# VachaLab/gorder

Hardware: AMD Instinct MI355X
Metric: trajectory frames/sec (higher is better)
Workload: dtype f32

## Files before the change

gorder_amd/abi.py:

```python
from __future__ import annotations

import ctypes as C
import os
from dataclasses import dataclass, field
from typing import List, Optional, Sequence

import numpy as np

_HERE = os.path.dirname(os.path.abspath(__file__))
LIB_PATH = os.environ.get("GORDER_HIP_LIB") or os.path.join(_HERE, "libgorder_hip.so")

OK = 0
ERR_UNDEFINED_BOX = 1
ERR_NOT_ORTHOGONAL_BOX = 2
ERR_ZERO_BOX = 3
ERR_UNDEFINED_POSITION = 4
ERR_INVALID_GLOBAL_MEMBRANE_CENTER = 5
ERR_INVALID_LOCAL_MEMBRANE_CENTER = 6
ERR_INVALID_ARGUMENT = 100
ERR_DEVICE = 101
ERR_NO_DEVICE = 102
ERR_BOX_RANGE = 103
ERR_LEAFLETS_NOT_PRIMED = 104
ERR_OVERFLOW = 105
# ... 235 lines not shown
        ge = self.geometry
        grp = _u32(ge.group) if ge.group is not None else None
        t.geometry.kind = ge.kind
        t.geometry.invert = 1 if ge.invert else 0
        t.geometry.reference = ge.reference
        t.geometry.point[:] = [float(x) for x in ge.point]
        t.geometry.n_group = 0 if grp is None else grp.size
        t.geometry.group = _ptr(grp)
        t.geometry.xdim[:] = [float(x) for x in ge.xdim]
        t.geometry.ydim[:] = [float(x) for x in ge.ydim]
        t.geometry.zdim[:] = [float(x) for x in ge.zdim]
        t.geometry.radius = ge.radius
        t.geometry.span[:] = [float(x) for x in ge.span]
        t.geometry.orientation = ge.orientation
        t.geometry.structure_box[:] = [float(x) for x in ge.structure_box]
        dn = self.dynamic_normal
        cloud = _u32(dn.cloud) if dn.cloud is not None else None
        t.dynamic_normal.enabled = 1 if dn.enabled else 0
        t.dynamic_normal.radius = dn.radius
        t.dynamic_normal.n_cloud = 0 if cloud is None else cloud.size
        t.dynamic_normal.cloud = _ptr(cloud)
        keep += [mts, mem, grp, cloud]
        return t, keep


_EXPORTS = [
    "gorder_hip_create", "gorder_hip_destroy", "gorder_hip_n_accumulators", "gorder_hip_ordermap_dims",
    "gorder_hip_set_stream", "gorder_hip_submit_device", "gorder_hip_submit_host",
    "gorder_hip_prime_leaflets", "gorder_hip_set_manual_leaflets", "gorder_hip_synchronize",
    "gorder_hip_finish", "gorder_hip_timewise", "gorder_hip_leaflets", "gorder_hip_leaflet_distances",
    "gorder_hip_normals", "gorder_hip_export_maps", "gorder_hip_set_normals",
    "gorder_hip_accumulators_device", "gorder_hip_bind_accumulators", "gorder_hip_last_error_index", "gorder_hip_last_error_frame", "gorder_hip_kernel_time_names",
    "gorder_hip_last_error_message", "gorder_hip_strerror", "gorder_hip_kernel_time", "gorder_hip_kernel_time_group", "gorder_hip_plan",
    "gorder_hip_plan_tables", "gorder_hip_selftest_arithmetic", "gorder_hip_selftest_trig", "gorder_hip_run_trajectory",
    "gorder_hip_comm_unique_id", "gorder_hip_comm_create", "gorder_hip_comm_destroy", "gorder_hip_allreduce",
    "gorder_hip_reset", "gorder_hip_xtc_decode", "gorder_hip_release_staging", "gorder_hip_speculation_stats", "gorder_hip_local_decide_stats",
]

_lib = None


class GorderHipError(RuntimeError):
    def __init__(self, status: int, message: str = "", index: int = 0, frame: int = 0):
        self.status = status
        self.index = index
        self.frame = frame
        super().__init__(f"gorder_hip status {status}: {message}")


def load_library() -> C.CDLL:
    global _lib
    if _lib is not None:
        return _lib
    if not os.path.exists(LIB_PATH):
        raise GorderHipError(ERR_NO_DEVICE, f"{LIB_PATH} is missing: run `python -c 'import __graft_entry__ as g; "
                                            "g.build()'` (there is no CPU fallback)")
    try:
        import torch
        _rt = os.path.join(os.path.dirname(torch.__file__), "lib", "libamdhip64.so")
        if os.path.exists(_rt):
            C.CDLL(_rt, mode=C.RTLD_GLOBAL)
    except ImportError:
        pass
    lib = C.CDLL(LIB_PATH)
    vp, u32, u64, i32 = C.c_void_p, C.c_uint32, C.c_uint64, C.c_int
    lib.gorder_hip_create.argtypes = [C.POINTER(CTables), C.POINTER(vp)]
    lib.gorder_hip_destroy.argtypes = [vp]
# ... 3 lines not shown
    lib.gorder_hip_ordermap_dims.argtypes = [vp, C.POINTER(u32), C.POINTER(u32)]
    lib.gorder_hip_ordermap_dims.restype = u32
    lib.gorder_hip_set_stream.argtypes = [vp, vp]
    lib.gorder_hip_submit_device.argtypes = [vp, vp, vp, vp, u32]
    lib.gorder_hip_submit_host.argtypes = [vp, vp, vp, vp, u32]
    lib.gorder_hip_prime_leaflets.argtypes = [vp, vp, vp, u64]
    lib.gorder_hip_set_manual_leaflets.argtypes = [vp, vp, u64]
    lib.gorder_hip_synchronize.argtypes = [vp]
    lib.gorder_hip_finish.argtypes = [vp, vp, vp, vp, vp, C.POINTER(u64)]
    lib.gorder_hip_timewise.argtypes = [vp, vp, vp, u64]
    lib.gorder_hip_leaflets.argtypes = [vp, vp, C.POINTER(u64)]
    lib.gorder_hip_leaflet_distances.argtypes = [vp, vp]
    lib.gorder_hip_normals.argtypes = [vp, vp, vp]
    lib.gorder_hip_export_maps.argtypes = [vp, vp, vp, u64]
    lib.gorder_hip_set_normals.argtypes = [vp, vp, u32]
    lib.gorder_hip_accumulators_device.argtypes = [vp, C.POINTER(vp), C.POINTER(u64)]
    lib.gorder_hip_bind_accumulators.argtypes = [vp, vp, u64]
    lib.gorder_hip_last_error_index.argtypes = [vp]
    lib.gorder_hip_last_error_index.restype = u64
    lib.gorder_hip_kernel_time_names.argtypes = [vp]
    lib.gorder_hip_kernel_time_names.restype = C.c_char_p
    lib.gorder_hip_last_error_frame.argtypes = [vp]
    lib.gorder_hip_last_error_frame.restype = u64
    lib.gorder_hip_last_error_message.argtypes = [vp]
    lib.gorder_hip_last_error_message.restype = C.c_char_p
    lib.gorder_hip_strerror.argtypes = [i32]
    lib.gorder_hip_strerror.restype = C.c_char_p
    lib.gorder_hip_kernel_time.argtypes = [vp, C.POINTER(C.c_double), C.POINTER(u64), i32]
    lib.gorder_hip_kernel_time_group.argtypes = [vp, C.c_uint32, C.POINTER(C.c_char_p), C.POINTER(C.c_double), C.POINTER(u64)]
    lib.gorder_hip_plan.argtypes = [vp, C.POINTER(CPlan)]
    lib.gorder_hip_speculation_stats.argtypes = [vp, C.POINTER(C.c_uint64)]
    lib.gorder_hip_local_decide_stats.argtypes = [vp, C.POINTER(C.c_uint64)]
    lib.gorder_hip_plan_tables.argtypes = [C.POINTER(CTables), C.POINTER(CPlan), C.POINTER(i32)]
    lib.gorder_hip_selftest_arithmetic.argtypes = [i32, C.c_uint64, C.c_uint64, C.POINTER(C.c_uint64)]
    lib.gorder_hip_selftest_trig.argtypes = [i32, i32, C.c_uint32, C.c_uint32, C.c_uint32, C.c_void_p]
    lib.gorder_hip_run_trajectory.argtypes = [vp, C.POINTER(CTrajectory), C.POINTER(CTrajectoryStats)]
    lib.gorder_hip_comm_unique_id.argtypes = [vp]
    lib.gorder_hip_comm_create.argtypes = [vp, vp, i32, i32, C.POINTER(vp)]
    lib.gorder_hip_comm_destroy.argtypes = [vp]
    lib.gorder_hip_comm_destroy.restype = None
    lib.gorder_hip_allreduce.argtypes = [vp, vp]
    lib.gorder_hip_reset.argtypes = [vp]
    lib.gorder_hip_xtc_decode.argtypes = [vp, vp, u64, vp, u32, u32, vp, u32, vp, u32]
    lib.gorder_hip_release_staging.argtypes = [vp]
    lib.gorder_hip_release_staging.restype = None
    _lib = lib
    return lib


def selftest_trig(fn: str, first_bits: int, stride: int, n: int, device: int = 0) -> np.ndarray:
    lib = load_library()
    out = np.empty(n, dtype=np.float32)
    st = lib.gorder_hip_selftest_trig(device, {"acos": 0, "acos_cores": 1, "cos": 2, "sin": 3}[fn], first_bits, stride, n, out.ctypes.data)
    if st != 0:
        raise GorderHipError(st, "gorder_hip_selftest_trig")
    return out


def selftest_arithmetic(n: int = 1 << 26, seed: int = 1, device: int = 0):
    lib = load_library()
    out = (C.c_uint64 * 2)()
    st = lib.gorder_hip_selftest_arithmetic(device, n, seed, out)
    if st != 0:
        raise GorderHipError(st, lib.gorder_hip_strerror(st).decode())
    return int(out[0]), int(out[1])


def plan_tables(tables: Tables) -> dict:
    lib = load_library()
    ct, keep = tables.as_ctypes()
    plan, check = CPlan(), C.c_int(-1)
    st = lib.gorder_hip_plan_tables(C.byref(ct), C.byref(plan), C.byref(check))
    if st != OK:
        raise GorderHipError(st, lib.gorder_hip_strerror(st).decode())
    d = {name: getattr(plan, name) for name, _ in CPlan._fields_}
    d["selfcheck"] = check.value
    return d


@dataclass
class Results:
    sums: np.ndarray
    counts: np.ndarray
    n_frames: int
    map_sums: Optional[np.ndarray] = None
    map_counts: Optional[np.ndarray] = None

    def order_ticks(self, min_samples: int = 1) -> np.ndarray:
        n = self.counts.astype(np.int64)
        ok = n >= max(1, min_samples)
        q = np.full(self.sums.shape, np.iinfo(np.int64).min, dtype=np.int64)
        q[ok] = (np.abs(self.sums[ok]) // n[ok]) * np.sign(self.sums[ok])
        return q

    def order(self, min_samples: int = 1) -> np.ndarray:
        out = np.full(self.sums.shape, np.nan, dtype=np.float32)
        n = self.counts.astype(np.int64)
        ok = n >= max(1, min_samples)
# ... 248 lines not shown
```

gorder_amd/csrc/gorder_hip.hip:

```cpp
#include <hip/hip_runtime.h>

#include <dlfcn.h>

#include <cmath>
#include <cstdio>
#include <cstdlib>
#include <cstring>
#include <mutex>
#include <new>
#include <string>
#include <deque>
#include <vector>

#include "../../include/gorder_hip.h"
#include "gm_math.h"
#include "plan.h"

#pragma clang fp contract(off)

using gorder::DirectItem;
using gorder::Item;
using gorder::kBlock;
using gorder::Plan;
using gorder::Tile;

#include "kernels_common.h"
#include "kernels_bonds.h"
#include "kernels_extras.h"
#include "kernels_leaflets.h"
#include "kernels_normals.h"
#include "kernels_xtc.h"


struct gorder_hip_handle {
    void *traj_cache = nullptr;
    void (*traj_cache_free)(gorder_hip_handle *) = nullptr;
    Plan plan;
    gorder_tables_t tables{};
    int device = 0;
    hipStream_t own_stream = nullptr;
    hipStream_t stream = nullptr;
    Tile *d_tiles = nullptr;
    Item *d_items = nullptr;
    uint32_t *d_tile_slots = nullptr;
    DirectItem *d_direct = nullptr;
    Tile *d_ua_tiles = nullptr;
    gorder::UaItem *d_ua_items = nullptr;
    uint32_t *d_ua_tile_slots = nullptr;
    uint32_t map_nx = 0, map_ny = 0;
    unsigned long long *d_map_sums = nullptr, *d_map_cnts = nullptr;
    unsigned long long *d_map_packed = nullptr;
    unsigned long long *d_map_rec = nullptr;
    size_t map_rec_cap = 0;
    gorder::MapRun *d_ua_runs = nullptr, *d_runs = nullptr;
// ... 63 lines not shown
    bool spec_enabled = false;
    bool spec_now = false;
    uint2 *d_own = nullptr;
    float4 *d_mom = nullptr;
    size_t mom_cap = 0;
    float *d_head_z = nullptr;
    size_t head_z_cap = 0;
    uint32_t *d_own_head_begin = nullptr;
    uint2 *d_own_heads = nullptr;
    float *d_spec_center = nullptr;
    uint8_t *d_spec_ok = nullptr;
    size_t spec_frames_cap = 0;
    uint32_t *d_spec_counters = nullptr;
    static constexpr uint32_t kSpecRing = 8;
    uint32_t *h_spec_counters = nullptr;
    hipEvent_t spec_counters_copied[kSpecRing] = {};
    uint64_t spec_ring_frames[kSpecRing] = {};
    uint32_t *d_spec_mol_begin = nullptr;
    SpecSample *d_spec_samples = nullptr;
    uint64_t spec_batches = 0, spec_fixed = 0, spec_exact_frames = 0;
    float *d_stage_xyz[2] = {nullptr, nullptr}, *d_stage_box[2] = {nullptr, nullptr};
    size_t stage_xyz_cap[2] = {0, 0}, stage_box_cap[2] = {0, 0};
    hipEvent_t stage_copied[2] = {nullptr, nullptr}, stage_computed[2] = {nullptr, nullptr};
    bool stage_used[2] = {false, false};
    int stage_next = 0;
    hipStream_t copy_stream = nullptr;
    float n2 = 1.0f, n2sq = 1.0f;
    int axis = -1;
    int frames_per_stage = kFramesPerStage;
    bool membrane_is_frame = false;
    bool use_gather = false;
    uint32_t wg_capacity = 256u * 6u;
    uint32_t wg_target = 0;
    uint32_t lw = 0;
    size_t lds_bytes = 0;
    uint64_t n_frames = 0;
    uint64_t err_index = 0;
    std::string err_msg;
    static constexpr uint32_t kTimingEvents = 1024;
    struct TimingSeg { uint32_t label, ev_a, ev_b; };
    bool timing_on = false;
    hipEvent_t timing_ev[kTimingEvents] = {};
    uint32_t timing_next_ev = 0;
    int timing_open_label = -1;
    uint32_t timing_open_ev = 0;
    std::deque<TimingSeg> timing_pending;
    std::vector<std::string> timing_labels;
    std::vector<double> timing_label_ms;
    std::vector<uint64_t> timing_label_n;
    uint64_t timing_launches = 0;
    std::string timed_kernels;
    std::vector<uint32_t> host_heads, host_dyn_heads;
    uint32_t *d_mol_slot0 = nullptr;
    uint64_t err_frame = 0;
    struct BatchLog { uint64_t ordinal, first, stride; std::vector<uint64_t> list; };
    static constexpr size_t kBatchLog = 4096;
    std::deque<BatchLog> batch_log;
    uint64_t n_submits = 0;
    const unsigned long long *decoder_key = nullptr;
};

namespace {

int fail(gorder_hip_handle *h, int status, const std::string &msg) {
    if (h) h->err_msg = msg;
    return status;
// ... 199 lines not shown
    HIP_TRY(h, hipGetLastError());
    h->last_normals.resize(4 * (size_t)n_mol);
    HIP_TRY(h, hipMemcpyAsync(h->last_normals.data(), h->d_dyn_normals + (size_t)(a.n_frames - 1) * n_mol,
                              4 * sizeof(float) * (size_t)n_mol, hipMemcpyDeviceToHost, h->stream));
    return GORDER_OK;
}

int launch_orders(gorder_hip_handle *h, FrameArgs &a) {
    const Plan &p = h->plan;
    const uint32_t n_tiles = (uint32_t)p.tiles.size();
    const bool extras = h->extra.maps || h->extra.tw || h->extra.geom_kind || h->dyn || h->manual_active;
#define name(k) TIMING_MARK(h, k)
    if (h->dyn && !h->manual_active) {
        const int st2 = run_dynamic_normals(h, a);
        if (st2 != GORDER_OK) return st2;
    }
    if (h->extra.geom_kind) {
        int st2;
        if ((st2 = ensure(h, &h->d_shapes, &h->shapes_cap, (size_t)a.n_frames * 8)) != GORDER_OK) return st2;
        const gorder_geometry_t &ge = h->tables.geometry;
        GeomArgs ga{};
        ga.xyz = a.xyz; ga.box9 = a.box9; ga.n_atoms = a.n_atoms; ga.pbc = a.pbc;
        ga.kind = ge.kind; ga.reference = ge.reference; ga.orientation = ge.orientation;
        for (int d = 0; d < 3; d++) { ga.point[d] = ge.point[d]; ga.structure_box[d] = ge.structure_box[d]; }
        for (int d = 0; d < 2; d++) { ga.xdim[d] = ge.xdim[d]; ga.ydim[d] = ge.ydim[d]; ga.zdim[d] = ge.zdim[d]; ga.span[d] = ge.span[d]; }
        ga.radius = ge.radius; ga.group = h->d_geom_group; ga.n_group = ge.n_group;
        ga.shapes = h->d_shapes; ga.err = h->d_err;
        name("k_geom_shapes");
        hipLaunchKernelGGL(k_geom_shapes, dim3(a.n_frames), dim3(256), 0, h->stream, ga);
        HIP_TRY(h, hipGetLastError());
    }
    if (n_tiles && !extras) {
        const uint32_t G = (uint32_t)h->frames_per_stage;
        const uint32_t n_stages = (a.n_frames + G - 1) / G;
        uint32_t target = h->wg_target ? h->wg_target : h->wg_capacity;
        if (!h->wg_target) target = 12u * h->wg_capacity;
        uint32_t n_chunks = std::max(1u, target / n_tiles);
        n_chunks = std::min(n_chunks, std::max(1u, n_stages / 4u));
        uint32_t fpc = ((n_stages + n_chunks - 1) / n_chunks) * G;
        n_chunks = (a.n_frames + fpc - 1) / fpc;
        a.frames_per_chunk = fpc;
        const uint64_t grid = (uint64_t)n_tiles * n_chunks;
        if (grid > 0x7fffffffull) return fail(h, GORDER_ERR_INVALID_ARGUMENT, "batch too large");
        const bool ac = (h->tables.flags & GORDER_FLAG_TRIG_ACOS_COS) != 0;
        const dim3 g((uint32_t)grid), b(kBlock);
#define GORDER_LAUNCH_TILED_A(G_, NPF_, AC_, PBC_, LF_, AX_)                                               \
        do {                                                                                                \
            if (LF_ && h->spec_now)                                                                         \
                hipLaunchKernelGGL((k_bonds_tiled<G_, NPF_, AC_, PBC_, LF_, AX_, LF_>), g, b, h->lds_bytes, h->stream, a, \
                                   a.xyz, a.box9, a.aflags, a.arow, h->d_tiles, h->d_items, h->d_tile_slots, n_tiles, h->lw); \
            else                                                                                            \
                hipLaunchKernelGGL((k_bonds_tiled<G_, NPF_, AC_, PBC_, LF_, AX_>), g, b, h->lds_bytes, h->stream, a,     \
                                   a.xyz, a.box9, a.aflags, a.arow, h->d_tiles, h->d_items, h->d_tile_slots, n_tiles,   \
                                   h->lw);                                                                  \
        } while (0)
#define GORDER_LAUNCH_TILED_V(G_, NPF_, AC_, PBC_, LF_)                                                    \
        do {                                                                                                \
            if (h->axis == 2) GORDER_LAUNCH_TILED_A(G_, NPF_, AC_, PBC_, LF_, 2);                           \
            else if (h->axis == 1) GORDER_LAUNCH_TILED_A(G_, NPF_, AC_, PBC_, LF_, 1);                      \
            else if (h->axis == 0) GORDER_LAUNCH_TILED_A(G_, NPF_, AC_, PBC_, LF_, 0);                      \
            else GORDER_LAUNCH_TILED_A(G_, NPF_, AC_, PBC_, LF_, -1);                                       \
        } while (0)
#define GORDER_LAUNCH_TILED(G_, NPF_)                                                                       \
        do {                                                                                                \
            const int v_ = (ac ? 4 : 0) | (a.pbc ? 2 : 0) | (a.leaflets ? 1 : 0);                           \
            switch (v_) {                                                                                   \
                case 0: GORDER_LAUNCH_TILED_V(G_, NPF_, false, false, false); break;                        \
                case 1: GORDER_LAUNCH_TILED_V(G_, NPF_, false, false, true); break;                         \
                case 2: GORDER_LAUNCH_TILED_V(G_, NPF_, false, true, false); break;                         \
                case 3: GORDER_LAUNCH_TILED_V(G_, NPF_, false, true, true); break;                          \
                case 4: GORDER_LAUNCH_TILED_V(G_, NPF_, true, false, false); break;                         \
                case 5: GORDER_LAUNCH_TILED_V(G_, NPF_, true, false, true); break;                          \
                case 6: GORDER_LAUNCH_TILED_V(G_, NPF_, true, true, false); break;                          \
                default: GORDER_LAUNCH_TILED_V(G_, NPF_, true, true, true); break;                          \
            }                                                                                               \
// ... 349 lines not shown
    if (device < 0 || device >= count || hipSetDevice(device) != hipSuccess) return GORDER_ERR_INVALID_ARGUMENT;
    if (n == 0) return GORDER_OK;
    float *d = nullptr;
    if (hipMalloc((void **)&d, (size_t)n * sizeof(float)) != hipSuccess) return GORDER_ERR_DEVICE;
    hipLaunchKernelGGL(k_selftest_trig, dim3((n + 255u) / 256u), dim3(256), 0, 0, fn, first_bits, stride, n, d);
    int st = GORDER_OK;
    if (hipDeviceSynchronize() != hipSuccess || hipMemcpy(out, d, (size_t)n * sizeof(float), hipMemcpyDeviceToHost) != hipSuccess)
        st = GORDER_ERR_DEVICE;
    (void)hipFree(d);
    return st;
}

int gorder_hip_plan_tables(const gorder_tables_t *tables, gorder_hip_plan_t *out, int *selfcheck) {
    if (!tables || !out) return GORDER_ERR_INVALID_ARGUMENT;
    Plan p;
    const int st = gorder::build_plan(*tables, env_flag("GORDER_HIP_FORCE_DIRECT"), p);
    if (st != GORDER_OK) return st;
    out->n_tiles = (uint32_t)p.tiles.size();
    out->block_threads = kBlock;
    out->max_window_atoms = p.max_window;
    out->n_direct_items = (uint32_t)p.direct.size();
    out->frames_per_stage = kFramesPerStage;
    const uint32_t lw = ((3u * p.max_window + 3u + 3u) / 4u) * 4u;
    size_t lds = (size_t)kFramesPerStage * lw * sizeof(float);
    if (lds < (size_t)kBlock * 24) lds = (size_t)kBlock * 24;
    out->lds_bytes = (uint32_t)lds;
    out->map_staged = 0;
    out->map_lds_bytes = 0;
    out->leaflets_one_read = p.spec_ok ? 1u : 0u;
    if (selfcheck) *selfcheck = gorder::selfcheck_plan(*tables, p);
    return GORDER_OK;
}

int gorder_hip_create(const gorder_tables_t *t, gorder_hip_handle **out) {
    if (!t || !out) return GORDER_ERR_INVALID_ARGUMENT;
    *out = nullptr;
    int n_dev = 0;
    if (hipGetDeviceCount(&n_dev) != hipSuccess || n_dev <= 0) return GORDER_ERR_NO_DEVICE;
    if (t->device < 0 || t->device >= n_dev) return GORDER_ERR_INVALID_ARGUMENT;

    gorder_hip_handle *h = new (std::nothrow) gorder_hip_handle();
    if (!h) return GORDER_ERR_DEVICE;
    *out = h;
    h->tables = *t;
    h->tables.molecule_types = nullptr;
    h->tables.leaflets.membrane = nullptr;
    h->device = t->device;
    HIP_TRY(h, hipSetDevice(h->device));
    if ((t->flags & GORDER_FLAG_UA_FAST_NORMALISE) && (t->flags & GORDER_FLAG_TRIG_ACOS_COS))
        return fail(h, GORDER_ERR_INVALID_ARGUMENT, "GORDER_FLAG_UA_FAST_NORMALISE (tolerance-bounded) and GORDER_FLAG_TRIG_ACOS_COS (literal) exclude each other");
    const bool ua_rows_only = t->timewise && !t->ordermap.enabled && t->geometry.kind == GORDER_GEOM_NONE && !t->dynamic_normal.enabled;
    int st = gorder::build_plan(*t, env_flag("GORDER_HIP_FORCE_DIRECT"), h->plan, !env_flag("GORDER_HIP_UA_SLOT_WAVES") && !ua_rows_only);
    if (st != GORDER_OK) return fail(h, st, "invalid bond tables");
    const Plan &p = h->plan;
    for (uint32_t m = 0; m < t->n_molecule_types; m++)
        h->map_max_mol = std::max(h->map_max_mol, t->molecule_types[m].n_molecules);
    HIP_TRY(h, hipStreamCreateWithFlags(&h->own_stream, hipStreamNonBlocking));
    h->stream = h->own_stream;
    if ((st = upload(h, &h->d_tiles, p.tiles)) != GORDER_OK) return st;
    if ((st = upload(h, &h->d_items, p.items)) != GORDER_OK) return st;
    if ((st = upload(h, &h->d_tile_slots, p.tile_slots)) != GORDER_OK) return st;
    if ((st = upload(h, &h->d_direct, p.direct)) != GORDER_OK) return st;
    if ((st = upload(h, &h->d_ua_tiles, p.ua_tiles)) != GORDER_OK) return st;
    if ((st = upload(h, &h->d_ua_items, p.ua_items)) != GORDER_OK) return st;
    if ((st = upload(h, &h->d_ua_tile_slots, p.ua_tile_slots)) != GORDER_OK) return st;
    {
// ... 65 lines not shown
        }
        if ((e.maps || e.tw || e.geom_kind) && !p.direct.empty())
            return fail(h, GORDER_ERR_INVALID_ARGUMENT,
                        "ordermaps / timewise / geometry need every bond to fit an atom window");
    }
    HIP_TRY(h, hipMalloc((void **)&h->d_err, (kErrWords + 2u) * sizeof(uint32_t)));
    HIP_TRY(h, hipMemset(h->d_err, 0xff, kErrWords * sizeof(uint32_t)));
    HIP_TRY(h, hipMemset(h->d_err + kErrWords, 0, 2u * sizeof(uint32_t)));
    h->acc_words = 4 * (size_t)p.n_acc + 1;
    HIP_TRY(h, hipMalloc((void **)&h->d_acc, h->acc_words * sizeof(unsigned long long)));
    HIP_TRY(h, hipMemset(h->d_acc, 0, h->acc_words * sizeof(unsigned long long)));
    if (const char *e = getenv("GORDER_HIP_MAP_FOLD_LIMIT")) {
        const long v = atol(e);
        if (v >= 2 && (unsigned long long)v <= kMapFoldLimit) h->map_fold_limit = (uint64_t)v;
    }
    if (const char *e = getenv("GORDER_HIP_REPLICAS")) {
        const int r = atoi(e);
        if (r >= 1 && r <= 1024) h->n_rep = (uint32_t)r;
    }
    if (p.n_acc) {
        const size_t rep_bytes = (size_t)h->n_rep * 4u * p.n_acc * sizeof(unsigned long long);
        HIP_TRY(h, hipMalloc((void **)&h->d_rep, rep_bytes));
        HIP_TRY(h, hipMemset(h->d_rep, 0, rep_bytes));
    }
    {
        const float *n = t->normal;
        h->n2sq = (n[0] * n[0] + n[1] * n[1]) + n[2] * n[2];
        h->n2 = sqrtf(h->n2sq);
        for (int d = 0; d < 3; d++)
            if (n[d] == 1.0f && n[(d + 1) % 3] == 0.0f && n[(d + 2) % 3] == 0.0f) h->axis = d;
        h->extra.axis = h->axis;
    }
    if (const char *e = getenv("GORDER_HIP_KERNEL")) h->use_gather = strcmp(e, "gather") == 0;
    if (const char *e = getenv("GORDER_HIP_WG_TARGET")) {
        const int w = atoi(e);
        if (w > 0) h->wg_target = (uint32_t)w;
    }
    h->lw = ((3u * p.max_window + 3u + 3u) / 4u) * 4u;
    h->lds_bytes = (size_t)h->frames_per_stage * h->lw * sizeof(float);
    if (h->lds_bytes < (size_t)kBlock * 24) h->lds_bytes = (size_t)kBlock * 24;
    {
        int n_cu = 256, per_cu = 6;
        (void)hipDeviceGetAttribute(&n_cu, hipDeviceAttributeMultiprocessorCount, h->device);
        const bool ac = (t->flags & GORDER_FLAG_TRIG_ACOS_COS) != 0;
        const hipError_t e = ac ? hipOccupancyMaxActiveBlocksPerMultiprocessor(&per_cu, k_bonds_tiled<4, 5, true, true, false, -1>, kBlock, h->lds_bytes)
                                : hipOccupancyMaxActiveBlocksPerMultiprocessor(&per_cu, k_bonds_tiled<4, 5, false, true, false, 2>, kBlock, h->lds_bytes);
        if (e != hipSuccess || per_cu < 1) per_cu = 4;
        h->wg_capacity = (uint32_t)n_cu * (uint32_t)per_cu;
    }

    const gorder_dynamic_normal_t &dn = t->dynamic_normal;
    if (dn.enabled) {
        if (!(dn.radius > 0.0f)) return fail(h, GORDER_ERR_INVALID_ARGUMENT, "dynamic normals need a positive radius");
        if (!dn.cloud || dn.n_cloud == 0) return fail(h, GORDER_ERR_INVALID_ARGUMENT, "dynamic normals need the NormalHeads group");
        if (!p.direct.empty()) return fail(h, GORDER_ERR_INVALID_ARGUMENT, "dynamic normals: a bond spans more than the LDS window");
        std::vector<uint32_t> cloud(dn.cloud, dn.cloud + dn.n_cloud), nheads;
        for (uint32_t a : cloud)
            if (a >= t->n_atoms) return fail(h, GORDER_ERR_INVALID_ARGUMENT, "NormalHeads index out of range");
        for (uint32_t m = 0; m < t->n_molecule_types; m++) {
            const gorder_moltype_t &mt = t->molecule_types[m];
            if (!mt.normal_heads) return fail(h, GORDER_ERR_INVALID_ARGUMENT, "dynamic normals need normal_heads[] per molecule type");
            for (uint32_t k = 0; k < mt.n_molecules; k++) {
                if (mt.normal_heads[k] >= t->n_atoms) return fail(h, GORDER_ERR_INVALID_ARGUMENT, "normal head index out of range");
                nheads.push_back(mt.normal_heads[k]);
            }
        }
// ... 942 lines not shown
```

gorder_amd/csrc/kernels_bonds.h:

```cpp
#pragma once

namespace {

__device__ __forceinline__ int grid_index(float x, float lo, float bin, uint32_t n, bool core) {
    const float k = __builtin_roundf(core ? gm_div_core(x - lo, bin) : (x - lo) / bin);
    if (!(k >= 0.0f) || !(k < (float)n)) return -1;
    return (int)k;
}
__device__ __forceinline__ int grid_index_fast(float x, float lo, float inv_bin, uint32_t n) {
    const float k = __builtin_floorf(__builtin_fmaf(x - lo, inv_bin, 0.5f));
    if (!(k >= 0.0f) || !(k < (float)n)) return -1;
    return (int)k;
}
constexpr uint32_t kRecFrames = 4;
struct TiledMapOut {
    uint32_t plane;
    float x0, y0, binx, biny;
    uint32_t nx, ny;
    int bin_core;
    unsigned long long *words;
    unsigned long long *ticks;
};
__device__ __forceinline__ unsigned long long tick_sample_word(int tick, bool lower) {
    return ((unsigned long long)(lower ? 1u : 0u) << 32) | (unsigned long long)(uint32_t)tick;
// ... 290 lines not shown
            s += d;
            q = __builtin_fmaf(d, d, q);
            mn = mom_min(mn, z[u]);
            mx = mom_max(mx, z[u]);
        }
    }
#define GORDER_MOM_STEP(CTRL, MASK, CTRL_TEXT)                                                  \
    s += mom_dpp0<CTRL, MASK>(s); q += mom_dpp0<CTRL, MASK>(q);                                 \
    GORDER_MOM_MINMAX_DPP(CTRL_TEXT);
    GORDER_MOM_STEP(0x111, 0xf, "row_shr:1 row_mask:0xf bank_mask:0xf")
    GORDER_MOM_STEP(0x112, 0xf, "row_shr:2 row_mask:0xf bank_mask:0xf")
    GORDER_MOM_STEP(0x114, 0xf, "row_shr:4 row_mask:0xf bank_mask:0xf")
    GORDER_MOM_STEP(0x118, 0xf, "row_shr:8 row_mask:0xf bank_mask:0xf")
    GORDER_MOM_STEP(0x142, 0xa, "row_bcast:15 row_mask:0xa bank_mask:0xf")
    GORDER_MOM_STEP(0x143, 0xc, "row_bcast:31 row_mask:0xc bank_mask:0xf")
#undef GORDER_MOM_STEP
    const bool all_finite = __all(finite);
    if (lane == 63u) a.mom[(size_t)f * n_tiles + tile_id] = make_float4(all_finite ? s : __builtin_nanf(""), q, mn, mx);
    if (my_head.y != 0xffffffffu) a.head_z[(size_t)f * a.n_mol_total + my_head.y] = slot[sh + a.mom_dim + 3u * my_head.x];
}
template <int G, int NPF, bool ACOS_COS, bool PBC, bool LEAF, int AXIS, bool MOM = false>
__global__ __launch_bounds__(kBlock, GORDER_TILED_MIN_WAVES) void k_bonds_tiled(FrameArgs a_in, const float *__restrict__ xyz,
                                                      const float *__restrict__ box9,
                                                      const uint8_t *__restrict__ aflags,
                                                      const uint32_t *__restrict__ arow,
                                                      const Tile *__restrict__ tiles,
                                                      const Item *__restrict__ items,
                                                      const uint32_t *__restrict__ tile_slots,
                                                      uint32_t n_tiles, uint32_t lw) {
    extern __shared__ __attribute__((aligned(16))) float lds[];
    using S = TiledStage<G, NPF, ACOS_COS, PBC, LEAF, AXIS>;
    FrameArgs a = a_in;
    a.xyz = xyz; a.box9 = box9; a.aflags = aflags; a.arow = arow;
    const uint32_t tile_id = blockIdx.x % n_tiles;
    const uint32_t chunk = blockIdx.x / n_tiles;
    const Tile t = tiles[tile_id];
    const uint32_t tid = threadIdx.x;
    const uint32_t sk = tid / S::TPF, si = tid % S::TPF;
    const bool active = tid < t.n_items;
    Item it{0, 0, 0, 0, 0};
    if (active) it = items[t.item0 + tid];

    const uint32_t f_begin = chunk * a.frames_per_chunk;
    const uint32_t f_end = min(a.n_frames, f_begin + a.frames_per_chunk);
    const uint32_t f_full = f_begin + ((f_end - f_begin) / G) * G;

    SampleAcc acc;
    int bad = 0;
    uint32_t nan_which = 0, nan_frame = kNoNan;
    v4f pre[NPF];
    uint2 own = make_uint2(0u, 0u), my_head = make_uint2(0u, 0xffffffffu);
    if (MOM) {
        own = a.own[tile_id];
        const uint32_t hq = a.own_head_begin[tile_id] + (tid & 63u);
        if (hq < a.own_head_begin[tile_id + 1u]) my_head = a.own_heads[hq];
    }

    if (f_begin < f_full) S::template load<false>(a, t, f_begin, f_end, sk, si, pre);
    for (uint32_t f0 = f_begin; f0 < f_full; f0 += G) {
        const bool finite = S::template store<false, MOM>(a, t, f0, f_end, sk, si, pre, lds, lw);
        __syncthreads();
        if (f0 + G < f_full) S::template load<false>(a, t, f0 + G, f_end, sk, si, pre);
        if (MOM) {
            static_assert(!MOM || (uint32_t)G * 64u == kBlock, "a wave per frame slot");
            tiled_moments(a, t, own, tile_id, n_tiles, f0 + sk, lds + (size_t)sk * lw, finite, my_head);
        }
        if (active) S::compute(a, t, it, f0, lds, lw, acc, bad, nan_which, nan_frame);
        __syncthreads();
    }
    if (f_full < f_end) {
        S::template load<true>(a, t, f_full, f_end, sk, si, pre);
        const bool finite = S::template store<true, MOM>(a, t, f_full, f_end, sk, si, pre, lds, lw);
        __syncthreads();
        if (MOM && f_full + sk < f_end) tiled_moments(a, t, own, tile_id, n_tiles, f_full + sk, lds + (size_t)sk * lw, finite, my_head);
        if (active) S::compute_tail(a, t, it, f_full, f_end, lds, lw, acc, bad, nan_which, nan_frame);
        __syncthreads();
    }
// ... 158 lines not shown
```

gorder_amd/csrc/kernels_common.h:

```cpp
#pragma once

namespace {

constexpr int kFramesPerStage = 4;
constexpr uint32_t kErrWords = 8;

struct FrameArgs {
    const float *xyz;
    const float *box9;
    uint32_t n_atoms;
    uint32_t n_frames;
    uint32_t frame0;
    uint32_t frames_per_chunk;
    int pbc;
    float nx, ny, nz, n2, n2sq;
    int leaflets;
    const uint8_t *aflags;
    const uint32_t *arow;
    uint32_t n_mol_total;
    unsigned long long *acc;
    unsigned long long *rep;
    uint32_t n_rep;
    uint32_t n_acc;
    uint32_t *err;
    const uint2 *own;
    float4 *mom;
    int mom_dim;
    const uint32_t *own_head_begin;
    const uint2 *own_heads;
    float *head_z;
};

constexpr unsigned long long kErrNone = ~0ull;
enum ErrStage : uint32_t { kStageBox = 0, kStageSystem = 1, kStageTypes = 2, kStageEnd = 3 };
__device__ __forceinline__ void raise_error(uint32_t *err, uint32_t code, uint32_t frame, uint32_t stage,
                                            uint32_t slot = 0, uint32_t sample = 0, uint32_t mol = 0,
                                            uint32_t detail = 0) {
    const unsigned long long key =
        ((unsigned long long)(code == GORDER_ERR_BOX_RANGE ? 1u : 0u) << 63) |
        ((unsigned long long)min(frame, 0x7fffffu) << 40) | ((unsigned long long)(stage & 3u) << 38) |
        ((unsigned long long)min(slot, 0x3fffu) << 24) | ((unsigned long long)(sample & 1u) << 23) |
        ((unsigned long long)min(mol, 0x1ffffu) << 6) | ((unsigned long long)(detail & 3u) << 4) |
        (unsigned long long)(code == GORDER_ERR_BOX_RANGE ? 8u : (code == GORDER_ERR_TRAJECTORY_FORMAT ? 9u : (code & 15u)));
    atomicMin(reinterpret_cast<unsigned long long *>(err), key);
}
__device__ __forceinline__ void raise_box_range(uint32_t *err, uint32_t frame) {
// ... 99 lines not shown
```

gorder_amd/csrc/plan.h:

```cpp
#pragma once
#include <algorithm>
#include <map>
#include <tuple>
#include <cstdint>
#include <utility>
#include <vector>

#include "../../include/gorder_hip.h"

namespace gorder {

#ifndef GORDER_BLOCK
#define GORDER_BLOCK 256
#endif
constexpr uint32_t kBlock = GORDER_BLOCK;
constexpr uint32_t kMaxWindow = 1024;

struct Item {
    uint16_t li, lj;
    uint16_t lslot;
    uint16_t pad;
    uint32_t mol;
};
struct Tile {
// ... 444 lines not shown
            for (uint32_t j = 0; j < run.n; j++) {
                const Item &it = p.items_by_slot[tile.item0 + run.tid0 + j];
                if (p.tile_slots[tile.slot0 + it.lslot] != sl) return 10;
                if (p.item_run.size() != p.items.size() || p.item_run[tile.item0 + run.tid0 + j] != ((run.tid0 << 16) | run.n))
                    return 16;
                covered[tile.item0 + run.tid0 + j]++;
            }
        }
    for (uint32_t c : covered)
        if (c != 1) return 11;
    if (!p.ua_tiles.empty()) {
        if (p.ua_run_begin.size() != (size_t)p.n_acc + 1) return 12;
        size_t lanes = 0, want_lanes = 0;
        for (const UaItem &it : p.ua_items) want_lanes += it.kind == GORDER_UA_CH3 ? 3 : it.kind == GORDER_UA_CH2 ? 2 : 1;
        for (uint32_t sl = 0; sl < p.n_acc; sl++)
            for (uint32_t r = p.ua_run_begin[sl]; r < p.ua_run_begin[sl + 1]; r++) {
                const MapRun &run = p.ua_runs[r];
                if (run.tile >= p.ua_tiles.size() || run.k > 2 || run.tid0 + run.n > p.ua_tiles[run.tile].n_items) return 13;
                const Tile &tile = p.ua_tiles[run.tile];
                for (uint32_t j = 0; j < run.n; j++) {
                    const UaItem &it = p.ua_items[tile.item0 + run.tid0 + j];
                    if (p.ua_tile_slots[tile.slot0 + it.lslot0 + run.k] != sl) return 14;
                    if (p.ua_item_run.size() != p.ua_items.size() ||
                        p.ua_item_run[tile.item0 + run.tid0 + j] != ((run.tid0 << 16) | run.n))
                        return 17;
                    lanes++;
                }
            }
        if (lanes != want_lanes) return 15;
    }
    return 0;
}

}
```

include/gorder_hip.h:

```cpp
#ifndef GORDER_HIP_H
#define GORDER_HIP_H

#include <stddef.h>
#include <stdint.h>

#include "gorder_xtc.h"

#ifdef __cplusplus
extern "C" {
#endif

typedef enum {
    GORDER_OK = 0,
    GORDER_ERR_UNDEFINED_BOX = 1,
    GORDER_ERR_NOT_ORTHOGONAL_BOX = 2,
    GORDER_ERR_ZERO_BOX = 3,
    GORDER_ERR_UNDEFINED_POSITION = 4,
    GORDER_ERR_INVALID_GLOBAL_MEMBRANE_CENTER = 5,
    GORDER_ERR_INVALID_LOCAL_MEMBRANE_CENTER = 6,
    GORDER_ERR_DYNAMIC_NORMAL = 7,
    GORDER_ERR_INVALID_ARGUMENT = 100,
    GORDER_ERR_DEVICE = 101,
    GORDER_ERR_NO_DEVICE = 102,
    GORDER_ERR_BOX_RANGE = 103,
// ... 176 lines not shown
int gorder_hip_comm_unique_id(uint8_t id[128]);
int gorder_hip_comm_create(gorder_hip_handle *h, const uint8_t id[128], int n_ranks, int rank, void **comm_out);
void gorder_hip_comm_destroy(void *comm);
int gorder_hip_allreduce(gorder_hip_handle *h, void *nccl_comm);

int gorder_hip_reset(gorder_hip_handle *h);

int gorder_hip_export_maps(gorder_hip_handle *h, void *d_sums, void *d_counts, uint64_t n_u64);

int gorder_hip_bind_accumulators(gorder_hip_handle *h, void *d_ptr, uint64_t n_u64);

uint64_t gorder_hip_last_error_index(const gorder_hip_handle *h);
uint64_t gorder_hip_last_error_frame(const gorder_hip_handle *h);
const char *gorder_hip_last_error_message(const gorder_hip_handle *h);
const char *gorder_hip_strerror(int status);

int gorder_hip_kernel_time(gorder_hip_handle *h, double *ms, uint64_t *launches, int reset);
int gorder_hip_kernel_time_group(gorder_hip_handle *h, uint32_t index, const char **name, double *ms, uint64_t *segments);
const char *gorder_hip_kernel_time_names(const gorder_hip_handle *h);

typedef struct {
    uint32_t n_tiles;
    uint32_t block_threads;
    uint32_t max_window_atoms;
    uint32_t n_direct_items;
    uint32_t frames_per_stage;
    uint32_t lds_bytes;
    uint32_t map_staged;
    uint32_t map_lds_bytes;
    uint32_t leaflets_one_read;
} gorder_hip_plan_t;
int gorder_hip_plan(const gorder_hip_handle *h, gorder_hip_plan_t *plan);
int gorder_hip_plan_tables(const gorder_tables_t *tables, gorder_hip_plan_t *plan, int *selfcheck);

int gorder_hip_speculation_stats(gorder_hip_handle *h, uint64_t out[4]);

int gorder_hip_local_decide_stats(gorder_hip_handle *h, uint64_t out[4]);

int gorder_hip_selftest_arithmetic(int device, uint64_t n, uint64_t seed, uint64_t mismatches[2]);
int gorder_hip_selftest_trig(int device, int fn, uint32_t first_bits, uint32_t stride, uint32_t n, float *out);

#ifdef __cplusplus
}
#endif
#endif
```

Measured before the change: 20.94 million.

## Balance tiled kernel chunks across XCDs with grouped work decomposition

Replaces the tile×chunk grid calculation with a scheduler that picks a chunk count that is a multiple of 8 (the XCD count) and minimizes wave-quantization waste against workgroup capacity. Stages are spread evenly, with the first n_long chunks taking one extra stage. Block indices are decoded so that consecutive blocks on different XCDs share a tile. The intent is to cut tail imbalance from uneven chunks and partial waves, and to improve per-XCD cache locality for tile data. The cost is extra integer decode per block and a more complex schedule; a legacy env option and a host-side inspection API are added.

```diff
diff --git a/gorder_amd/abi.py b/gorder_amd/abi.py
--- a/gorder_amd/abi.py
+++ b/gorder_amd/abi.py
@@ -291,7 +291,7 @@
     "gorder_hip_normals", "gorder_hip_export_maps", "gorder_hip_set_normals",
     "gorder_hip_accumulators_device", "gorder_hip_bind_accumulators", "gorder_hip_last_error_index", "gorder_hip_last_error_frame", "gorder_hip_kernel_time_names",
     "gorder_hip_last_error_message", "gorder_hip_strerror", "gorder_hip_kernel_time", "gorder_hip_kernel_time_group", "gorder_hip_plan",
-    "gorder_hip_plan_tables", "gorder_hip_selftest_arithmetic", "gorder_hip_selftest_trig", "gorder_hip_run_trajectory",
+    "gorder_hip_plan_tables", "gorder_hip_tiled_schedule", "gorder_hip_selftest_arithmetic", "gorder_hip_selftest_trig", "gorder_hip_run_trajectory",
     "gorder_hip_comm_unique_id", "gorder_hip_comm_create", "gorder_hip_comm_destroy", "gorder_hip_allreduce",
     "gorder_hip_reset", "gorder_hip_xtc_decode", "gorder_hip_release_staging", "gorder_hip_speculation_stats", "gorder_hip_local_decide_stats",
 ]
@@ -361,6 +361,7 @@
     lib.gorder_hip_speculation_stats.argtypes = [vp, C.POINTER(C.c_uint64)]
     lib.gorder_hip_local_decide_stats.argtypes = [vp, C.POINTER(C.c_uint64)]
     lib.gorder_hip_plan_tables.argtypes = [C.POINTER(CTables), C.POINTER(CPlan), C.POINTER(i32)]
+    lib.gorder_hip_tiled_schedule.argtypes = [u32, u32, u32, u32, i32, vp, vp, u64]
     lib.gorder_hip_selftest_arithmetic.argtypes = [i32, C.c_uint64, C.c_uint64, C.POINTER(C.c_uint64)]
     lib.gorder_hip_selftest_trig.argtypes = [i32, i32, C.c_uint32, C.c_uint32, C.c_uint32, C.c_void_p]
     lib.gorder_hip_run_trajectory.argtypes = [vp, C.POINTER(CTrajectory), C.POINTER(CTrajectoryStats)]
@@ -393,6 +394,23 @@
     if st != 0:
         raise GorderHipError(st, lib.gorder_hip_strerror(st).decode())
     return int(out[0]), int(out[1])
+
+
+def k1_schedule(n_frames: int, n_tiles: int, capacity: int, target: int = 0, legacy: bool = False, launches: bool = False):
+    lib = load_library()
+    info = np.zeros(5, dtype=np.uint32)
+    st = lib.gorder_hip_tiled_schedule(n_frames, n_tiles, capacity, target, int(legacy), info.ctypes.data, None, 0)
+    if st != OK:
+        raise GorderHipError(st, lib.gorder_hip_strerror(st).decode())
+    d = dict(zip(("n_chunks", "stages", "n_long", "grouped", "grid"), (int(v) for v in info)))
+    if launches:
+        out = np.zeros((d["grid"], 3), dtype=np.uint32)
+        st = lib.gorder_hip_tiled_schedule(n_frames, n_tiles, capacity, target, int(legacy), info.ctypes.data,
+                                        out.ctypes.data, d["grid"])
+        if st != OK:
+            raise GorderHipError(st, lib.gorder_hip_strerror(st).decode())
+        d["launches"] = out
+    return d
 
 
 def plan_tables(tables: Tables) -> dict:
diff --git a/gorder_amd/csrc/gorder_hip.hip b/gorder_amd/csrc/gorder_hip.hip
--- a/gorder_amd/csrc/gorder_hip.hip
+++ b/gorder_amd/csrc/gorder_hip.hip
@@ -20,6 +20,7 @@
 
 using gorder::DirectItem;
 using gorder::Item;
+using gorder::k1_decode;
 using gorder::kBlock;
 using gorder::Plan;
 using gorder::Tile;
@@ -149,6 +150,7 @@
     bool use_gather = false;
     uint32_t wg_capacity = 256u * 6u;
     uint32_t wg_target = 0;
+    bool k1_legacy = false;
     uint32_t lw = 0;
     size_t lds_bytes = 0;
     uint64_t n_frames = 0;
@@ -414,15 +416,12 @@
     }
     if (n_tiles && !extras) {
         const uint32_t G = (uint32_t)h->frames_per_stage;
-        const uint32_t n_stages = (a.n_frames + G - 1) / G;
-        uint32_t target = h->wg_target ? h->wg_target : h->wg_capacity;
-        if (!h->wg_target) target = 12u * h->wg_capacity;
-        uint32_t n_chunks = std::max(1u, target / n_tiles);
-        n_chunks = std::min(n_chunks, std::max(1u, n_stages / 4u));
-        uint32_t fpc = ((n_stages + n_chunks - 1) / n_chunks) * G;
-        n_chunks = (a.n_frames + fpc - 1) / fpc;
-        a.frames_per_chunk = fpc;
-        const uint64_t grid = (uint64_t)n_tiles * n_chunks;
+        const uint32_t target = h->wg_target ? h->wg_target : 12u * h->wg_capacity;
+        const gorder::K1Schedule ks = gorder::k1_schedule(a.n_frames, G, n_tiles, h->wg_capacity, target,
+                                                          h->k1_legacy || h->use_gather);
+        a.frames_per_chunk = ks.stages * G;
+        a.n_chunks = ks.n_chunks; a.chunk_stages = ks.stages; a.n_long = ks.n_long; a.grouped = ks.grouped;
+        const uint64_t grid = ks.grid;
         if (grid > 0x7fffffffull) return fail(h, GORDER_ERR_INVALID_ARGUMENT, "batch too large");
         const bool ac = (h->tables.flags & GORDER_FLAG_TRIG_ACOS_COS) != 0;
         const dim3 g((uint32_t)grid), b(kBlock);
@@ -838,6 +837,25 @@
     return GORDER_OK;
 }
 
+int gorder_hip_tiled_schedule(uint32_t n_frames, uint32_t n_tiles, uint32_t capacity, uint32_t target, int legacy,
+                           uint32_t *info, uint32_t *launches, uint64_t max_launches) {
+    if (!info) return GORDER_ERR_INVALID_ARGUMENT;
+    const uint32_t G = kFramesPerStage;
+    const gorder::K1Schedule s = gorder::k1_schedule(n_frames, G, n_tiles, capacity, target ? target : 12u * capacity, legacy != 0);
+    info[0] = s.n_chunks; info[1] = s.stages; info[2] = s.n_long; info[3] = s.grouped;
+    info[4] = (uint32_t)std::min<uint64_t>(s.grid, 0xffffffffu);
+    if (!launches) return GORDER_OK;
+    if (s.grid > max_launches) return GORDER_ERR_INVALID_ARGUMENT;
+    for (uint32_t L = 0; L < (uint32_t)s.grid; L++) {
+        uint32_t tile = 0, f0 = 0, f1 = 0;
+        const bool on = k1_decode(L, n_tiles, G, n_frames, s.n_chunks, s.stages, s.n_long, s.grouped, tile, f0, f1);
+        launches[3u * (size_t)L] = on ? tile : 0xffffffffu;
+        launches[3u * (size_t)L + 1] = f0;
+        launches[3u * (size_t)L + 2] = f1;
+    }
+    return GORDER_OK;
+}
+
 int gorder_hip_create(const gorder_tables_t *t, gorder_hip_handle **out) {
     if (!t || !out) return GORDER_ERR_INVALID_ARGUMENT;
     *out = nullptr;
@@ -969,6 +987,7 @@
         h->extra.axis = h->axis;
     }
     if (const char *e = getenv("GORDER_HIP_KERNEL")) h->use_gather = strcmp(e, "gather") == 0;
+    if (const char *e = getenv("GORDER_HIP_K1_SCHEDULE")) h->k1_legacy = strcmp(e, "legacy") == 0;
     if (const char *e = getenv("GORDER_HIP_WG_TARGET")) {
         const int w = atoi(e);
         if (w > 0) h->wg_target = (uint32_t)w;
diff --git a/gorder_amd/csrc/kernels_bonds.h b/gorder_amd/csrc/kernels_bonds.h
--- a/gorder_amd/csrc/kernels_bonds.h
+++ b/gorder_amd/csrc/kernels_bonds.h
@@ -346,8 +346,10 @@
     using S = TiledStage<G, NPF, ACOS_COS, PBC, LEAF, AXIS>;
     FrameArgs a = a_in;
     a.xyz = xyz; a.box9 = box9; a.aflags = aflags; a.arow = arow;
-    const uint32_t tile_id = blockIdx.x % n_tiles;
-    const uint32_t chunk = blockIdx.x / n_tiles;
+    uint32_t tile_id, f_begin, f_end;
+    if (!k1_decode(blockIdx.x, n_tiles, (uint32_t)G, a.n_frames, a.n_chunks, a.chunk_stages, a.n_long, a.grouped, tile_id,
+                   f_begin, f_end))
+        return;
     const Tile t = tiles[tile_id];
     const uint32_t tid = threadIdx.x;
     const uint32_t sk = tid / S::TPF, si = tid % S::TPF;
@@ -355,8 +357,6 @@
     Item it{0, 0, 0, 0, 0};
     if (active) it = items[t.item0 + tid];
 
-    const uint32_t f_begin = chunk * a.frames_per_chunk;
-    const uint32_t f_end = min(a.n_frames, f_begin + a.frames_per_chunk);
     const uint32_t f_full = f_begin + ((f_end - f_begin) / G) * G;
 
     SampleAcc acc;
diff --git a/gorder_amd/csrc/kernels_common.h b/gorder_amd/csrc/kernels_common.h
--- a/gorder_amd/csrc/kernels_common.h
+++ b/gorder_amd/csrc/kernels_common.h
@@ -12,6 +12,7 @@
     uint32_t n_frames;
     uint32_t frame0;
     uint32_t frames_per_chunk;
+    uint32_t n_chunks, chunk_stages, n_long, grouped;
     int pbc;
     float nx, ny, nz, n2, n2sq;
     int leaflets;
diff --git a/gorder_amd/csrc/plan.h b/gorder_amd/csrc/plan.h
--- a/gorder_amd/csrc/plan.h
+++ b/gorder_amd/csrc/plan.h
@@ -500,4 +500,76 @@
     return 0;
 }
 
-}
+#if defined(__HIP__)
+#define GORDER_HD __host__ __device__
+#else
+#define GORDER_HD
+#endif
+constexpr uint32_t kXcds = 8;
+struct K1Schedule {
+    uint32_t n_chunks = 0;
+    uint32_t stages = 0;
+    uint32_t n_long = 0;
+    uint32_t grouped = 0;
+    uint64_t grid = 0;
+};
+inline uint32_t gcd_u32(uint32_t a, uint32_t b) {
+    while (b) { const uint32_t r = a % b; a = b; b = r; }
+    return a;
+}
+inline K1Schedule k1_schedule(uint32_t n_frames, uint32_t G, uint32_t n_tiles, uint32_t capacity, uint32_t target, bool legacy) {
+    K1Schedule s;
+    if (!n_frames || !n_tiles || !G) return s;
+    const uint32_t n_stages = (n_frames + G - 1) / G;
+    const uint32_t c_max = std::max(1u, n_stages / 4u);
+    const uint32_t c0 = std::min(std::max(1u, target / n_tiles), c_max);
+    const uint64_t cap = std::max(1u, capacity);
+    auto waste = [&](uint32_t c) {
+        const uint64_t wg = (uint64_t)n_tiles * c;
+        return (double)((wg + cap - 1) / cap * cap) / (double)wg;
+    };
+    const uint32_t st = (n_stages + c0 - 1) / c0;
+    s.n_chunks = (n_stages + st - 1) / st;
+    s.stages = st;
+    s.grid = (uint64_t)n_tiles * s.n_chunks;
+    if (legacy || c0 < kXcds) return s;
+    uint32_t best = 0;
+    double best_waste = 0.0;
+    const uint32_t hi = std::max(kXcds, std::min(c_max, c0 + c0 / 4u) / kXcds * kXcds);
+    const uint32_t lo = std::min(hi, std::max(kXcds, (c0 - c0 / 4u + kXcds - 1u) / kXcds * kXcds));
+    for (uint32_t c = lo; c <= hi; c += kXcds) {
+        const double w = waste(c);
+        const uint32_t dist = c > c0 ? c - c0 : c0 - c, best_dist = best > c0 ? best - c0 : c0 - best;
+        if (!best || w < best_waste - 1e-9 || (w < best_waste + 1e-9 && dist < best_dist)) {
+            best = c;
+            best_waste = w;
+        }
+    }
+    if (best_waste > waste(s.n_chunks) + 0.05) return s;
+    s.n_chunks = best;
+    s.stages = n_stages / best;
+    s.n_long = n_stages % best;
+    s.grouped = 1;
+    s.grid = (uint64_t)n_tiles * best;
+    return s;
+}
+GORDER_HD inline bool k1_decode(uint32_t L, uint32_t n_tiles, uint32_t G, uint32_t n_frames, uint32_t n_chunks,
+                                uint32_t stages, uint32_t n_long, uint32_t grouped, uint32_t &tile, uint32_t &f_begin,
+                                uint32_t &f_end) {
+    uint32_t chunk;
+    if (grouped) {
+        const uint32_t r = L / kXcds;
+        chunk = (r / n_tiles) * kXcds + L % kXcds;
+        tile = r % n_tiles;
+    } else {
+        chunk = L / n_tiles;
+        tile = L % n_tiles;
+    }
+    if (chunk >= n_chunks) return false;
+    f_begin = G * (chunk * stages + (chunk < n_long ? chunk : n_long));
+    const uint32_t len = G * (stages + (chunk < n_long ? 1u : 0u));
+    f_end = n_frames - f_begin < len ? n_frames : f_begin + len;
+    return true;
+}
+
+}
diff --git a/include/gorder_hip.h b/include/gorder_hip.h
--- a/include/gorder_hip.h
+++ b/include/gorder_hip.h
@@ -232,6 +232,8 @@
 } gorder_hip_plan_t;
 int gorder_hip_plan(const gorder_hip_handle *h, gorder_hip_plan_t *plan);
 int gorder_hip_plan_tables(const gorder_tables_t *tables, gorder_hip_plan_t *plan, int *selfcheck);
+int gorder_hip_tiled_schedule(uint32_t n_frames, uint32_t n_tiles, uint32_t capacity, uint32_t target, int legacy,
+                           uint32_t *info, uint32_t *launches, uint64_t max_launches);
 
 int gorder_hip_speculation_stats(gorder_hip_handle *h, uint64_t out[4]);
 
```

After: 21.02 million, median of 4. No clear change (+0.4%).
